# Ye-zixiao/Double-YOLO-Kaist

Measured on AMD Instinct MI355X. Metric: paired RGB+LWIR images/sec (train step), higher is better.
Workload: dtype bf16; 1 GPU; kaist_dyolov4_fshare_global_concat_se3.cfg train step (fwd+loss+bwd+Adam), 640x512 pairs, batch 16/GPU; global_batch=16, parallelism=dp1

## Files before the change

### double-yolo-kaist_amd/csrc/bn_act.hip

```cpp
#include <stdlib.h>
#include "dyk_common.h"

namespace {

__global__ __launch_bounds__(256) void bn_finalize_kernel(DykFinPair pr) {
    const DykBnFinalizeDesc d = pr.d[blockIdx.z];
    const int sub = threadIdx.x & 31;
    const int c = blockIdx.x * (blockDim.x >> 5) + (threadIdx.x >> 5);
    if (c >= d.C) return;
    const double n = (double)d.count;
    const int slots = d.slots > 0 ? d.slots : 1;
    double s1 = 0.0, s2 = 0.0;
    for (int r = sub; r < slots; r += 32) {
        double* st = d.stats + (size_t)r * 2 * d.C;
        s1 += st[c]; s2 += st[d.C + c];
        st[c] = 0.0; st[d.C + c] = 0.0;
    }
#pragma unroll
    for (int o = 16; o > 0; o >>= 1) { s1 += __shfl_xor(s1, o, 64); s2 += __shfl_xor(s2, o, 64); }
    if (sub != 0) return;
    const double mean = s1 / n;
    double var = s2 / n - mean * mean;
    if (var < 0.0) var = 0.0;
    const float rstd = (float)(1.0 / sqrt(var + (double)d.eps));
    const float g = d.gamma ? d.gamma[c] : 1.f, b = d.beta ? d.beta[c] : 0.f;
    const float sc = g * rstd;
    d.scale[c] = sc;
    d.shift[c] = b - (float)mean * sc;
    if (d.save_mean) d.save_mean[c] = (float)mean;
    if (d.save_rstd) d.save_rstd[c] = rstd;
    if (d.running_mean) {
        const double unb = n > 1.0 ? var * n / (n - 1.0) : var;
        d.running_mean[c] = (1.f - d.momentum) * d.running_mean[c] + d.momentum * (float)mean;
        d.running_var[c] = (1.f - d.momentum) * d.running_var[c] + d.momentum * (float)unb;
    }
}

__global__ void bn_fold_kernel(const float* gamma, const float* beta, const float* rm, const float* rv, float eps,
                               float* scale, float* shift, int C) {
    const int c = blockIdx.x * blockDim.x + threadIdx.x;
    if (c >= C) return;
    const float sc = (gamma ? gamma[c] : 1.f) / sqrtf(rv[c] + eps);
    scale[c] = sc;
    shift[c] = (beta ? beta[c] : 0.f) - rm[c] * sc;
}

template <typename T, int ACT>
__global__ __launch_bounds__(256) void bn_act_fwd_kernel(DykEwPair pr, int CVB) {
    const DykEwDesc d = pr.d[blockIdx.z];
    constexpr int EPV = ElemTraits<T>::EPV;
    const int PY = 256 / CVB;
    const int tx = threadIdx.x % CVB, ty = threadIdx.x / CVB;
    const int cv = blockIdx.x * CVB + tx;
    if (cv * EPV >= d.C) return;
    const int c = cv * EPV;
    float sc[EPV], sh[EPV];
#pragma unroll
    for (int j = 0; j < EPV; ++j) { sc[j] = d.p0 ? d.p0[c + j] : 1.f; sh[j] = d.p1 ? d.p1[c + j] : 0.f; }
    const T* __restrict__ a = (const T*)d.a;
    const T* __restrict__ r = (const T*)d.b;
    T* __restrict__ o = (T*)d.out;
    constexpr int U = 4;
    const long chunk = ((d.npix + gridDim.y - 1) / gridDim.y + PY - 1) / PY * PY;
    const long pend = min((long)d.npix, ((long)blockIdx.y + 1) * chunk);
    const long pstep = PY;
    for (long p0 = (long)blockIdx.y * chunk + ty; p0 < pend; p0 += pstep * U) {
        uint4 vx[U], vr[U];
#pragma unroll
        for (int u = 0; u < U; ++u) {
            const long p = p0 + u * pstep;
            if (p < pend) {
                vx[u] = ld_stream16(a + p * d.lda + c);
                if (r) vr[u] = *(const uint4*)(r + p * d.ldb + c);
            }
        }
#pragma unroll
        for (int u = 0; u < U; ++u) {
            const long p = p0 + u * pstep;
            if (p >= pend) break;
            float x[EPV], y[EPV];
            vec_unpack<T>(vx[u], x);
#pragma unroll
            for (int j = 0; j < EPV; ++j) y[j] = act_fwd_c<ACT>(x[j] * sc[j] + sh[j]);
            if (r) {
                float rr[EPV];
                vec_unpack<T>(vr[u], rr);
#pragma unroll
                for (int j = 0; j < EPV; ++j) y[j] += rr[j];
            }
            *(uint4*)(o + p * d.ldo + c) = vec_pack<T>(y);
        }
    }
}

template <typename T, int ACT>
__global__ __launch_bounds__(256) void bn_fused_fwd_kernel(DykFinPair fp, DykEwPair pr, int CVB) {
    const DykBnFinalizeDesc f = fp.d[blockIdx.z];
    const DykEwDesc d = pr.d[blockIdx.z];
    constexpr int EPV = ElemTraits<T>::EPV;
    __shared__ float s_aff[2][256];
    const int PY = 256 / CVB;
    const int tx = threadIdx.x % CVB, ty = threadIdx.x / CVB;
    const int cv = blockIdx.x * CVB + tx;
    {
        const int c_base = blockIdx.x * CVB * EPV;
        const int nch = min(CVB * EPV, d.C - c_base);
        const int slots = f.slots > 0 ? f.slots : 1;
        const size_t rs = (size_t)2 * f.C;
        for (int cl = threadIdx.x; cl < nch; cl += 256) {
            const int c = c_base + cl;
            constexpr int FB = 16;
            double a1[4] = {0.0, 0.0, 0.0, 0.0}, a2[4] = {0.0, 0.0, 0.0, 0.0};
            int r = 0;
            for (; r + FB <= slots; r += FB) {
                double v1[FB], v2[FB];
#pragma unroll
                for (int u = 0; u < FB; ++u) { v1[u] = f.stats[(size_t)(r + u) * rs + c]; v2[u] = f.stats[(size_t)(r + u) * rs + f.C + c]; }
#pragma unroll
                for (int u = 0; u < FB; ++u) { a1[u & 3] += v1[u]; a2[u & 3] += v2[u]; }
            }
            for (; r + 4 <= slots; r += 4) {
#pragma unroll
                for (int u = 0; u < 4; ++u) { a1[u] += f.stats[(size_t)(r + u) * rs + c]; a2[u] += f.stats[(size_t)(r + u) * rs + f.C + c]; }
            }
            for (; r < slots; ++r) { a1[0] += f.stats[(size_t)r * rs + c]; a2[0] += f.stats[(size_t)r * rs + f.C + c]; }
            const double n = (double)f.count;
            const double mean = ((a1[0] + a1[1]) + (a1[2] + a1[3])) / n;
            double var = ((a2[0] + a2[1]) + (a2[2] + a2[3])) / n - mean * mean;
            if (var < 0.0) var = 0.0;
            const float rstd = (float)(1.0 / sqrt(var + (double)f.eps));
            const float g = f.gamma ? f.gamma[c] : 1.f, b = f.beta ? f.beta[c] : 0.f;
            const float sc = g * rstd, sh = b - (float)mean * sc;
            s_aff[0][cl] = sc;
            s_aff[1][cl] = sh;
            if (blockIdx.y == 0) {
                f.scale[c] = sc;
                f.shift[c] = sh;
                if (f.save_mean) f.save_mean[c] = (float)mean;
                if (f.save_rstd) f.save_rstd[c] = rstd;
                if (f.running_mean) {
                    const double unb = n > 1.0 ? var * n / (n - 1.0) : var;
                    f.running_mean[c] = (1.f - f.momentum) * f.running_mean[c] + f.momentum * (float)mean;
                    f.running_var[c] = (1.f - f.momentum) * f.running_var[c] + f.momentum * (float)unb;
                }
            }
        }
        __syncthreads();
    }
    if (cv * EPV >= d.C) return;
    const int c = cv * EPV;
    float sc[EPV], sh[EPV];
#pragma unroll
    for (int j = 0; j < EPV; ++j) { sc[j] = s_aff[0][tx * EPV + j]; sh[j] = s_aff[1][tx * EPV + j]; }
    const T* __restrict__ a = (const T*)d.a;
    const T* __restrict__ r = (const T*)d.b;
    T* __restrict__ o = (T*)d.out;
    constexpr int U = 4;
    const long chunk = ((d.npix + gridDim.y - 1) / gridDim.y + PY - 1) / PY * PY;
    const long pend = min((long)d.npix, ((long)blockIdx.y + 1) * chunk);
    const long pstep = PY;
    for (long p0 = (long)blockIdx.y * chunk + ty; p0 < pend; p0 += pstep * U) {
        uint4 vx[U], vr[U];
#pragma unroll
        for (int u = 0; u < U; ++u) {
            const long p = p0 + u * pstep;
            if (p < pend) {
                vx[u] = ld_stream16(a + p * d.lda + c);
                if (r) vr[u] = *(const uint4*)(r + p * d.ldb + c);
            }
        }
#pragma unroll
        for (int u = 0; u < U; ++u) {
            const long p = p0 + u * pstep;
            if (p >= pend) break;
            float x[EPV], y[EPV];
            vec_unpack<T>(vx[u], x);
#pragma unroll
            for (int j = 0; j < EPV; ++j) y[j] = act_fwd_c<ACT>(x[j] * sc[j] + sh[j]);
            if (r) {
                float rr[EPV];
                vec_unpack<T>(vr[u], rr);
#pragma unroll
                for (int j = 0; j < EPV; ++j) y[j] += rr[j];
            }
            *(uint4*)(o + p * d.ldo + c) = vec_pack<T>(y);
        }
    }
}

template <typename T, int ACT>
__global__ __launch_bounds__(256) void bn_act_bwd_reduce_kernel(DykEwPair pr, int CVB) {
    const DykEwDesc d = pr.d[blockIdx.z];
    constexpr int EPV = ElemTraits<T>::EPV;
    __shared__ float red[256 * 2 * 8];
    const int PY = 256 / CVB;
    const int tx = threadIdx.x % CVB, ty = threadIdx.x / CVB;
    const int CV = d.C / EPV;
    const int cv = blockIdx.x * CVB + tx;
    const int c = cv * EPV;
    const bool active = cv < CV;
    float s1[EPV], s2[EPV];
#pragma unroll
    for (int j = 0; j < EPV; ++j) s1[j] = s2[j] = 0.f;
    if (active) {
        float sc[EPV], sh[EPV], mu[EPV], rs[EPV];
#pragma unroll
        for (int j = 0; j < EPV; ++j) {
            sc[j] = d.p0[c + j]; sh[j] = d.p1[c + j]; mu[j] = d.p2[c + j]; rs[j] = d.p3[c + j];
        }
        const T* __restrict__ dz = (const T*)d.a;
        const T* __restrict__ y = (const T*)d.b;
        constexpr int U = 4;
        const long chunk = ((d.npix + gridDim.y - 1) / gridDim.y + PY - 1) / PY * PY;
            const long pend = min((long)d.npix, ((long)blockIdx.y + 1) * chunk);
            const long pstep = PY;
            for (long p0 = (long)blockIdx.y * chunk + ty; p0 < pend; p0 += pstep * U) {
            uint4 vg[U], vy[U];
#pragma unroll
            for (int u = 0; u < U; ++u) {
                const long p = p0 + u * pstep;
                if (p < pend) { vg[u] = ld_stream16(dz + p * d.lda + c); vy[u] = ld_stream16(y + p * d.ldb + c); }
            }
#pragma unroll
            for (int u = 0; u < U; ++u) {
                if (p0 + u * pstep >= pend) break;
                float g[EPV], yy[EPV];
                vec_unpack<T>(vg[u], g);
                vec_unpack<T>(vy[u], yy);
#pragma unroll
                for (int j = 0; j < EPV; ++j) {
                    const float da = g[j] * act_bwd_c<ACT>(yy[j] * sc[j] + sh[j]);
                    s1[j] += da;
                    s2[j] += da * ((yy[j] - mu[j]) * rs[j]);
                }
            }
        }
    }
    float* mine = red + threadIdx.x * 2 * 8;
#pragma unroll
    for (int j = 0; j < EPV; ++j) { mine[j] = s1[j]; mine[8 + j] = s2[j]; }
    __syncthreads();
    if (ty == 0 && active) {
        for (int q = 1; q < PY; ++q) {
            const float* o = red + (q * CVB + tx) * 2 * 8;
#pragma unroll
            for (int j = 0; j < EPV; ++j) { s1[j] += o[j]; s2[j] += o[8 + j]; }
        }
        double* rd = d.red + (size_t)(blockIdx.y % (unsigned)(d.slots > 0 ? d.slots : 1)) * 2 * d.C;
#pragma unroll
        for (int j = 0; j < EPV; ++j) {
            atomicAdd(rd + c + j, (double)s1[j]);
            atomicAdd(rd + d.C + c + j, (double)s2[j]);
        }
    }
}

__global__ __launch_bounds__(256) void bn_bwd_params_kernel(double* red, float* dgamma, float* dbeta, int C, int slots) {
    const int sub = threadIdx.x & 31;
    const int c = blockIdx.x * (blockDim.x >> 5) + (threadIdx.x >> 5);
    if (c >= C) return;
    double s1 = 0.0, s2 = 0.0;
    for (int r = sub; r < slots; r += 32) { s1 += red[(size_t)r * 2 * C + c]; s2 += red[(size_t)r * 2 * C + C + c]; }
#pragma unroll
    for (int o = 16; o > 0; o >>= 1) { s1 += __shfl_xor(s1, o, 64); s2 += __shfl_xor(s2, o, 64); }
    if (sub != 0) return;
    red[c] = s1; red[C + c] = s2;
    if (dbeta) dbeta[c] += (float)s1;
    if (dgamma) dgamma[c] += (float)s2;
}

template <typename T, int ACT>
__global__ __launch_bounds__(256) void bn_act_bwd_apply_kernel(DykEwPair pr, int CVB) {
    const DykEwDesc d = pr.d[blockIdx.z];
    constexpr int EPV = ElemTraits<T>::EPV;
    __shared__ float s_tot[2][256];
    const int PY = 256 / CVB;
    const int tx = threadIdx.x % CVB, ty = threadIdx.x / CVB;
    const int cv = blockIdx.x * CVB + tx;
    {
        const int c_base = blockIdx.x * CVB * EPV;
        const int nch = min(CVB * EPV, d.C - c_base);
        const int slots = d.slots > 0 ? d.slots : 1;
        const size_t rs = d.H > 0 ? (size_t)d.H : (size_t)2 * d.C;
        const size_t so = d.W > 0 ? (size_t)d.W : (size_t)d.C;
        for (int cl = threadIdx.x; cl < nch; cl += 256) {
            const double* p = d.red + c_base + cl;
            double a8[2][8] = {{0.0, 0.0, 0.0, 0.0, 0.0, 0.0, 0.0, 0.0}, {0.0, 0.0, 0.0, 0.0, 0.0, 0.0, 0.0, 0.0}};
            int r = 0;
            for (; r + 16 <= slots; r += 16) {
                double v[2][16];
#pragma unroll
                for (int u = 0; u < 16; ++u) { v[0][u] = p[(size_t)(r + u) * rs]; v[1][u] = p[(size_t)(r + u) * rs + so]; }
#pragma unroll
                for (int u = 0; u < 16; ++u) { a8[0][u & 7] += v[0][u]; a8[1][u & 7] += v[1][u]; }
            }
            for (; r + 8 <= slots; r += 8) {
#pragma unroll
                for (int u = 0; u < 8; ++u) { a8[0][u] += p[(size_t)(r + u) * rs]; a8[1][u] += p[(size_t)(r + u) * rs + so]; }
            }
            for (; r < slots; ++r) { a8[0][0] += p[(size_t)r * rs]; a8[1][0] += p[(size_t)r * rs + so]; }
#pragma unroll
            for (int which = 0; which < 2; ++which) {
                const double acc = ((a8[which][0] + a8[which][1]) + (a8[which][2] + a8[which][3])) + ((a8[which][4] + a8[which][5]) + (a8[which][6] + a8[which][7]));
                s_tot[which][cl] = (float)acc;
                if (blockIdx.y == 0) {
                    float* g = which ? (float*)d.aux : (float*)d.aux2;
                    if (g) g[c_base + cl] += (float)acc;
                }
            }
        }
        __syncthreads();
    }
    if (cv * EPV >= d.C) return;
    const int c = cv * EPV;
    const float invn = 1.f / (float)d.npix;
    float sc[EPV], sh[EPV], mu[EPV], rs[EPV], m1[EPV], m2[EPV];
#pragma unroll
    for (int j = 0; j < EPV; ++j) {
        sc[j] = d.p0[c + j]; sh[j] = d.p1[c + j]; mu[j] = d.p2[c + j]; rs[j] = d.p3[c + j];
        m1[j] = s_tot[0][tx * EPV + j] * invn; m2[j] = s_tot[1][tx * EPV + j] * invn;
    }
    const T* __restrict__ dz = (const T*)d.a;
    const T* __restrict__ y = (const T*)d.b;
    T* __restrict__ o = (T*)d.out;
    const bool accum = d.flags & DYK_EW_ACCUM;
    constexpr int U = 4;
    const long chunk = ((d.npix + gridDim.y - 1) / gridDim.y + PY - 1) / PY * PY;
    const long pend = min((long)d.npix, ((long)blockIdx.y + 1) * chunk);
    const long pstep = PY;
    for (long p0 = (long)blockIdx.y * chunk + ty; p0 < pend; p0 += pstep * U) {
        uint4 vg[U], vy[U], vo[U];
#pragma unroll
        for (int u = 0; u < U; ++u) {
            const long p = p0 + u * pstep;
            if (p < pend) {
                vg[u] = ld_stream16(dz + p * d.lda + c);
                vy[u] = ld_stream16(y + p * d.ldb + c);
                if (accum) vo[u] = *(const uint4*)(o + p * d.ldo + c);
            }
        }
#pragma unroll
        for (int u = 0; u < U; ++u) {
            const long p = p0 + u * pstep;
            if (p >= pend) break;
            float g[EPV], yy[EPV], r[EPV];
            vec_unpack<T>(vg[u], g);
            vec_unpack<T>(vy[u], yy);
#pragma unroll
            for (int j = 0; j < EPV; ++j) {
                const float da = g[j] * act_bwd_c<ACT>(yy[j] * sc[j] + sh[j]);
                const float xh = (yy[j] - mu[j]) * rs[j];
                r[j] = sc[j] * (da - m1[j] - xh * m2[j]);
            }
            if (accum) {
                float old[EPV];
                vec_unpack<T>(vo[u], old);
#pragma unroll
                for (int j = 0; j < EPV; ++j) r[j] += old[j];
            }
            *(uint4*)(o + p * d.ldo + c) = vec_pack<T>(r);
        }
    }
}

inline int ew_grid2d(int CV, long npix, int* gx, int* gy) {
    int CVB = 1;
    while (CVB < CV && CVB < 32) CVB <<= 1;
    const int PY = 256 / CVB;
    *gx = (CV + CVB - 1) / CVB;
    constexpr int ppt = 8, capb = 2048;
    long g = (npix + (long)PY * ppt - 1) / ((long)PY * ppt);
    const long cap = capb / *gx > 0 ? capb / *gx : 1;
    if (g > cap) g = cap;
    if (g < 1) g = 1;
    *gy = (int)g;
    return CVB;
}

#define DYK_BN_LAUNCH_ACT(KERNEL, T, ...)                                                                         \
    switch (d->act) {                                                                                              \
    case DYK_ACT_LINEAR: hipLaunchKernelGGL((KERNEL<T, DYK_ACT_LINEAR>), __VA_ARGS__); break;                      \
    case DYK_ACT_LEAKY: hipLaunchKernelGGL((KERNEL<T, DYK_ACT_LEAKY>), __VA_ARGS__); break;                        \
    case DYK_ACT_MISH: hipLaunchKernelGGL((KERNEL<T, DYK_ACT_MISH>), __VA_ARGS__); break;                          \
    case DYK_ACT_RELU: hipLaunchKernelGGL((KERNEL<T, DYK_ACT_RELU>), __VA_ARGS__); break;                          \
    case DYK_ACT_RELU6: hipLaunchKernelGGL((KERNEL<T, DYK_ACT_RELU6>), __VA_ARGS__); break;                        \
    case DYK_ACT_HSIGMOID: hipLaunchKernelGGL((KERNEL<T, DYK_ACT_HSIGMOID>), __VA_ARGS__); break;                  \
    case DYK_ACT_HSWISH: hipLaunchKernelGGL((KERNEL<T, DYK_ACT_HSWISH>), __VA_ARGS__); break;                      \
    default: return DYK_ERR_ARG;                                                                                   \
    }
#define DYK_BN_LAUNCH(KERNEL, ...)                                        \
    if (d->dtype == DYK_BF16) { DYK_BN_LAUNCH_ACT(KERNEL, bf16_t, __VA_ARGS__) } \
    else { DYK_BN_LAUNCH_ACT(KERNEL, float, __VA_ARGS__) }

inline int ew_check(const DykEwDesc* d, bool need_b) {
    if (!d || !d->a || !d->out || d->npix <= 0 || d->C <= 0) return DYK_ERR_ARG;
    if (need_b && !d->b) return DYK_ERR_ARG;
    const int epv = d->dtype == DYK_BF16 ? 8 : 4;
    if (d->dtype != DYK_BF16 && d->dtype != DYK_F32) return DYK_ERR_ARG;
    if (d->C % epv || d->lda % epv || d->ldo % epv || (d->b && d->ldb % epv)) return DYK_ERR_ARG;
    return DYK_OK;
}

}

extern "C" int dyk_bn_finalize(const DykBnFinalizeDesc* d, void* stream) {
    if (!d || !d->stats || !d->scale || !d->shift || d->C <= 0 || d->count <= 0) return DYK_ERR_ARG;
    DykFinPair fp;
    const int nz = dyk_fill_fin_pair(fp, d);
    if (!nz) return DYK_ERR_ARG;
    hipLaunchKernelGGL(bn_finalize_kernel, dim3((d->C + 7) / 8, 1, nz), dim3(256), 0, (hipStream_t)stream, fp);
    DYK_LAUNCH_CHECK();
    return DYK_OK;
}

extern "C" int dyk_bn_fold(const float* gamma, const float* beta, const float* running_mean,
                           const float* running_var, float eps, float* scale, float* shift, int32_t C,
                           void* stream) {
    if (!running_mean || !running_var || !scale || !shift || C <= 0) return DYK_ERR_ARG;
    hipLaunchKernelGGL(bn_fold_kernel, dim3((C + 127) / 128), dim3(128), 0, (hipStream_t)stream, gamma, beta,
                       running_mean, running_var, eps, scale, shift, C);
    DYK_LAUNCH_CHECK();
    return DYK_OK;
}

extern "C" int dyk_bn_act_fwd(const DykEwDesc* d, void* stream) {
    const int rc = ew_check(d, false);
    if (rc) return rc;
    const int epv = d->dtype == DYK_BF16 ? 8 : 4;
    int gx, gy;
    const int CVB = ew_grid2d(d->C / epv, d->npix, &gx, &gy);
    DykEwPair pr;
    const int nz = dyk_fill_ew_pair(pr, d);
    if (!nz) return DYK_ERR_ARG;
    DYK_BN_LAUNCH(bn_act_fwd_kernel, dim3(gx, gy, nz), dim3(256), 0, (hipStream_t)stream, pr, CVB)
    DYK_LAUNCH_CHECK();
    return DYK_OK;
}

extern "C" int dyk_bn_finalize_act_fwd(const DykBnFinalizeDesc* f, const DykEwDesc* d, void* stream) {
    if (!f || !f->stats || !f->scale || !f->shift || f->C <= 0 || f->count <= 0) return DYK_ERR_ARG;
    const int rc = ew_check(d, false);
    if (rc) return rc;
    if (d->C != f->C) return DYK_ERR_ARG;
    const int epv = d->dtype == DYK_BF16 ? 8 : 4;
    int gx, gy;
    const int CVB = ew_grid2d(d->C / epv, d->npix, &gx, &gy);
    DykEwPair pr;
    DykFinPair fp;
    const int nz = dyk_fill_ew_pair(pr, d);
    if (!nz || dyk_fill_fin_pair(fp, f) != nz) return DYK_ERR_ARG;
    DYK_BN_LAUNCH(bn_fused_fwd_kernel, dim3(gx, gy, nz), dim3(256), 0, (hipStream_t)stream, fp, pr, CVB)
    DYK_LAUNCH_CHECK();
    return DYK_OK;
}

extern "C" int dyk_bn_act_bwd_reduce(const DykEwDesc* d, void* stream) {
    if (!d || !d->a || !d->b || !d->red || !d->p0 || !d->p1 || !d->p2 || !d->p3) return DYK_ERR_ARG;
    if (d->npix <= 0 || d->C <= 0 || (d->dtype != DYK_BF16 && d->dtype != DYK_F32)) return DYK_ERR_ARG;
    const int epv = d->dtype == DYK_BF16 ? 8 : 4;
    if (d->C % epv || d->lda % epv || d->ldb % epv) return DYK_ERR_ARG;
    const int CV = d->C / epv;
    int CVB = 1;
    while (CVB < CV && CVB < 32) CVB <<= 1;
    const int PY = 256 / CVB;
    const int gx = (CV + CVB - 1) / CVB;
    long gy = ((long)d->npix + PY * 8 - 1) / (PY * 8);
    const long cap = 2048 / gx > 0 ? 2048 / gx : 1;
    if (gy > cap) gy = cap;
    if (gy < 1) gy = 1;
    DykEwPair pr;
    const int nz = dyk_fill_ew_pair(pr, d);
    if (!nz) return DYK_ERR_ARG;
    DYK_BN_LAUNCH(bn_act_bwd_reduce_kernel, dim3(gx, (int)gy, nz), dim3(256), 0, (hipStream_t)stream, pr, CVB)
    DYK_LAUNCH_CHECK();
    return DYK_OK;
}

extern "C" int dyk_bn_bwd_params(double* red, float* dgamma, float* dbeta, int32_t C, int32_t slots, void* stream) {
    if (!red || C <= 0) return DYK_ERR_ARG;
    hipLaunchKernelGGL(bn_bwd_params_kernel, dim3((C + 7) / 8), dim3(256), 0, (hipStream_t)stream, red, dgamma, dbeta, C,
                       slots > 0 ? slots : 1);
    DYK_LAUNCH_CHECK();
    return DYK_OK;
}

extern "C" int dyk_bn_act_bwd_apply(const DykEwDesc* d, void* stream) {
    const int rc = ew_check(d, true);
    if (rc) return rc;
    if (d->flags & DYK_EW_SKIP) return DYK_OK;
    if (!d->red || !d->p0 || !d->p1 || !d->p2 || !d->p3) return DYK_ERR_ARG;
    const int epv = d->dtype == DYK_BF16 ? 8 : 4;
    int gx, gy;
    const int CVB = ew_grid2d(d->C / epv, d->npix, &gx, &gy);
    DykEwPair pr;
    const int nz = dyk_fill_ew_pair(pr, d);
    if (!nz) return DYK_ERR_ARG;
    DYK_BN_LAUNCH(bn_act_bwd_apply_kernel, dim3(gx, gy, nz), dim3(256), 0, (hipStream_t)stream, pr, CVB)
    DYK_LAUNCH_CHECK();
    return DYK_OK;
}
```

Measured before the change: 583.1 pairs/s.

## Split BN stat replica folding across lanes and prefetch activations before finalize

In the fused BN finalize+activation forward kernel and the BN backward apply kernel, the per-channel reduction over stat replica slots is now spread across several lanes per channel (chosen at launch as 8, 4 or 1), with partial sums combined by cross-lane shuffles. When multiple lanes are used, the first activation tile loads, and in backward the per-channel parameters, are issued before the slot reduction so their latency overlaps it. The main loop is restructured into a request/compute pipeline that prefetches the next tile. The aim is to shorten the serial prologue in which only a few threads walked all slots, at the cost of more template variants, higher register pressure from the in-flight loads, and a changed floating-point summation order.

New measurement: 584.2 pairs/s (median of 3 runs). No clear change (+0.2%).

```diff
diff --git a/double-yolo-kaist_amd/csrc/bn_act.hip b/double-yolo-kaist_amd/csrc/bn_act.hip
--- a/double-yolo-kaist_amd/csrc/bn_act.hip
+++ b/double-yolo-kaist_amd/csrc/bn_act.hip
@@ -93,7 +93,72 @@
     }
 }
 
-template <typename T, int ACT>
+template <int NCH, int L, int NB>
+__device__ __forceinline__ void fold_batch(const double* __restrict__ p, size_t rs, size_t so, int r, uint32_t lo, double (&a)[2][NCH / L]) {
+    constexpr int K = NCH / L, PB = NB / NCH;
+    double v[2][K][PB];
+#pragma unroll
+    for (int i = 0; i < PB; ++i)
+#pragma unroll
+        for (int k = 0; k < K; ++k) {
+            const double* pr = p + (size_t)(r + i * NCH + k * L) * rs;
+            v[0][k][i] = pr[lo]; v[1][k][i] = (pr + so)[lo];
+        }
+#pragma unroll
+    for (int i = 0; i < PB; ++i)
+#pragma unroll
+        for (int k = 0; k < K; ++k) { a[0][k] += v[0][k][i]; a[1][k] += v[1][k][i]; }
+}
+
+template <int L>
+__device__ __forceinline__ void fold_lane(size_t rs, int& cl, int& q, uint32_t& lo) {
+    constexpr int CW = 64 / L;
+    const int lane = threadIdx.x & 63;
+    q = lane / CW;
+    cl = (threadIdx.x >> 6) * CW + lane % CW;
+    lo = (uint32_t)cl + (uint32_t)q * (uint32_t)rs;
+    if constexpr (L > 1) asm volatile("" : "+v"(lo));
+}
+
+template <int NCH, int L, int FB>
+__device__ __forceinline__ void fold_replicas(const double* __restrict__ p, size_t rs, size_t so, int slots, uint32_t lo, int q, bool live,
+                                              double& t0, double& t1) {
+    static_assert(NCH % L == 0 && FB % NCH == 0 && FB / NCH <= 8, "chains per lane, batches of whole rounds of the chains");
+    constexpr int K = NCH / L;
+    double a[2][K];
+#pragma unroll
+    for (int k = 0; k < K; ++k) a[0][k] = a[1][k] = 0.0;
+    if (live) {
+        const int whole = slots & ~(NCH - 1);
+        int r = 0;
+        if constexpr (L > 1) {
+            if (FB <= whole) {
+                fold_batch<NCH, L, FB>(p, rs, so, 0, lo, a);
+                for (r = FB; r + FB <= whole; r += FB) fold_batch<NCH, L, FB>(p, rs, so, r, lo, a);
+            }
+        } else {
+            for (; r + FB <= whole; r += FB) fold_batch<NCH, L, FB>(p, rs, so, r, lo, a);
+        }
+        if constexpr (FB / 2 >= NCH) if (r + FB / 2 <= whole) { fold_batch<NCH, L, FB / 2>(p, rs, so, r, lo, a); r += FB / 2; }
+        if constexpr (FB / 4 >= NCH) if (r + FB / 4 <= whole) { fold_batch<NCH, L, FB / 4>(p, rs, so, r, lo, a); r += FB / 4; }
+        if constexpr (FB / 8 >= NCH) if (r + FB / 8 <= whole) { fold_batch<NCH, L, FB / 8>(p, rs, so, r, lo, a); r += FB / 8; }
+        if (q == 0)
+            for (; r < slots; ++r) { a[0][0] += (p + (size_t)r * rs)[lo]; a[1][0] += (p + (size_t)r * rs + so)[lo]; }
+    }
+#pragma unroll
+    for (int m = 1; m < NCH; m <<= 1) {
+        if (m < L) {
+#pragma unroll
+            for (int k = 0; k < K; ++k) { a[0][k] += __shfl_xor(a[0][k], m * (64 / L), 64); a[1][k] += __shfl_xor(a[1][k], m * (64 / L), 64); }
+        } else {
+#pragma unroll
+            for (int k = 0; k < K; k += 2 * (m / L)) { a[0][k] += a[0][k + m / L]; a[1][k] += a[1][k + m / L]; }
+        }
+    }
+    t0 = a[0][0]; t1 = a[1][0];
+}
+
+template <typename T, int ACT, int L>
 __global__ __launch_bounds__(256) void bn_fused_fwd_kernel(DykFinPair fp, DykEwPair pr, int CVB) {
     const DykBnFinalizeDesc f = fp.d[blockIdx.z];
     const DykEwDesc d = pr.d[blockIdx.z];
@@ -102,56 +167,11 @@
     const int PY = 256 / CVB;
     const int tx = threadIdx.x % CVB, ty = threadIdx.x / CVB;
     const int cv = blockIdx.x * CVB + tx;
-    {
-        const int c_base = blockIdx.x * CVB * EPV;
-        const int nch = min(CVB * EPV, d.C - c_base);
-        const int slots = f.slots > 0 ? f.slots : 1;
-        const size_t rs = (size_t)2 * f.C;
-        for (int cl = threadIdx.x; cl < nch; cl += 256) {
-            const int c = c_base + cl;
-            constexpr int FB = 16;
-            double a1[4] = {0.0, 0.0, 0.0, 0.0}, a2[4] = {0.0, 0.0, 0.0, 0.0};
-            int r = 0;
-            for (; r + FB <= slots; r += FB) {
-                double v1[FB], v2[FB];
-#pragma unroll
-                for (int u = 0; u < FB; ++u) { v1[u] = f.stats[(size_t)(r + u) * rs + c]; v2[u] = f.stats[(size_t)(r + u) * rs + f.C + c]; }
-#pragma unroll
-                for (int u = 0; u < FB; ++u) { a1[u & 3] += v1[u]; a2[u & 3] += v2[u]; }
-            }
-            for (; r + 4 <= slots; r += 4) {
-#pragma unroll
-                for (int u = 0; u < 4; ++u) { a1[u] += f.stats[(size_t)(r + u) * rs + c]; a2[u] += f.stats[(size_t)(r + u) * rs + f.C + c]; }
-            }
-            for (; r < slots; ++r) { a1[0] += f.stats[(size_t)r * rs + c]; a2[0] += f.stats[(size_t)r * rs + f.C + c]; }
-            const double n = (double)f.count;
-            const double mean = ((a1[0] + a1[1]) + (a1[2] + a1[3])) / n;
-            double var = ((a2[0] + a2[1]) + (a2[2] + a2[3])) / n - mean * mean;
-            if (var < 0.0) var = 0.0;
-            const float rstd = (float)(1.0 / sqrt(var + (double)f.eps));
-            const float g = f.gamma ? f.gamma[c] : 1.f, b = f.beta ? f.beta[c] : 0.f;
-            const float sc = g * rstd, sh = b - (float)mean * sc;
-            s_aff[0][cl] = sc;
-            s_aff[1][cl] = sh;
-            if (blockIdx.y == 0) {
-                f.scale[c] = sc;
-                f.shift[c] = sh;
-                if (f.save_mean) f.save_mean[c] = (float)mean;
-                if (f.save_rstd) f.save_rstd[c] = rstd;
-                if (f.running_mean) {
-                    const double unb = n > 1.0 ? var * n / (n - 1.0) : var;
-                    f.running_mean[c] = (1.f - f.momentum) * f.running_mean[c] + f.momentum * (float)mean;
-                    f.running_var[c] = (1.f - f.momentum) * f.running_var[c] + f.momentum * (float)unb;
-                }
-            }
-        }
-        __syncthreads();
-    }
-    if (cv * EPV >= d.C) return;
     const int c = cv * EPV;
-    float sc[EPV], sh[EPV];
-#pragma unroll
-    for (int j = 0; j < EPV; ++j) { sc[j] = s_aff[0][tx * EPV + j]; sh[j] = s_aff[1][tx * EPV + j]; }
+    const bool active = c < d.C;
+    int cl, q;
+    uint32_t lo;
+    fold_lane<L>((size_t)2 * f.C, cl, q, lo);
     const T* __restrict__ a = (const T*)d.a;
     const T* __restrict__ r = (const T*)d.b;
     T* __restrict__ o = (T*)d.out;
@@ -159,8 +179,9 @@
     const long chunk = ((d.npix + gridDim.y - 1) / gridDim.y + PY - 1) / PY * PY;
     const long pend = min((long)d.npix, ((long)blockIdx.y + 1) * chunk);
     const long pstep = PY;
-    for (long p0 = (long)blockIdx.y * chunk + ty; p0 < pend; p0 += pstep * U) {
-        uint4 vx[U], vr[U];
+    long p0 = (long)blockIdx.y * chunk + ty;
+    uint4 vx[U], vr[U];
+    auto request = [&]() {
 #pragma unroll
         for (int u = 0; u < U; ++u) {
             const long p = p0 + u * pstep;
@@ -169,6 +190,53 @@
                 if (r) vr[u] = *(const uint4*)(r + p * d.ldb + c);
             }
         }
+    };
+    constexpr bool early = L > 1;
+    if (early && active) request();
+    {
+        const int c_base = blockIdx.x * CVB * EPV;
+        const int nch = min(CVB * EPV, d.C - c_base);
+        const int slots = f.slots > 0 ? f.slots : 1;
+        const bool live = cl < nch;
+        const int cf = c_base + cl;
+        float g = 1.f, b = 0.f;
+        float rm = 0.f, rv = 0.f;
+        if (live && q == 0) {
+            if (f.gamma) g = f.gamma[cf];
+            if (f.beta) b = f.beta[cf];
+            if (blockIdx.y == 0 && f.running_mean) { rm = f.running_mean[cf]; rv = f.running_var[cf]; }
+        }
+        double t1, t2;
+        fold_replicas<4, L, (L == 1 ? 16 : 32)>(f.stats + c_base, (size_t)2 * f.C, (size_t)f.C, slots, lo, q, live, t1, t2);
+        if (live && q == 0) {
+            const double n = (double)f.count;
+            const double mean = t1 / n;
+            double var = t2 / n - mean * mean;
+            if (var < 0.0) var = 0.0;
+            const float rstd = (float)(1.0 / sqrt(var + (double)f.eps));
+            const float sc = g * rstd, sh = b - (float)mean * sc;
+            s_aff[0][cl] = sc;
+            s_aff[1][cl] = sh;
+            if (blockIdx.y == 0) {
+                f.scale[cf] = sc;
+                f.shift[cf] = sh;
+                if (f.save_mean) f.save_mean[cf] = (float)mean;
+                if (f.save_rstd) f.save_rstd[cf] = rstd;
+                if (f.running_mean) {
+                    const double unb = n > 1.0 ? var * n / (n - 1.0) : var;
+                    f.running_mean[cf] = (1.f - f.momentum) * rm + f.momentum * (float)mean;
+                    f.running_var[cf] = (1.f - f.momentum) * rv + f.momentum * (float)unb;
+                }
+            }
+        }
+        __syncthreads();
+    }
+    if (!active) return;
+    float sc[EPV], sh[EPV];
+#pragma unroll
+    for (int j = 0; j < EPV; ++j) { sc[j] = s_aff[0][tx * EPV + j]; sh[j] = s_aff[1][tx * EPV + j]; }
+    if (!early) request();
+    while (p0 < pend) {
 #pragma unroll
         for (int u = 0; u < U; ++u) {
             const long p = p0 + u * pstep;
@@ -185,6 +253,8 @@
             }
             *(uint4*)(o + p * d.ldo + c) = vec_pack<T>(y);
         }
+        p0 += pstep * U;
+        request();
     }
 }
 
@@ -269,7 +339,7 @@
     if (dgamma) dgamma[c] += (float)s2;
 }
 
-template <typename T, int ACT>
+template <typename T, int ACT, int L>
 __global__ __launch_bounds__(256) void bn_act_bwd_apply_kernel(DykEwPair pr, int CVB) {
     const DykEwDesc d = pr.d[blockIdx.z];
     constexpr int EPV = ElemTraits<T>::EPV;
@@ -277,49 +347,13 @@
     const int PY = 256 / CVB;
     const int tx = threadIdx.x % CVB, ty = threadIdx.x / CVB;
     const int cv = blockIdx.x * CVB + tx;
-    {
-        const int c_base = blockIdx.x * CVB * EPV;
-        const int nch = min(CVB * EPV, d.C - c_base);
-        const int slots = d.slots > 0 ? d.slots : 1;
-        const size_t rs = d.H > 0 ? (size_t)d.H : (size_t)2 * d.C;
-        const size_t so = d.W > 0 ? (size_t)d.W : (size_t)d.C;
-        for (int cl = threadIdx.x; cl < nch; cl += 256) {
-            const double* p = d.red + c_base + cl;
-            double a8[2][8] = {{0.0, 0.0, 0.0, 0.0, 0.0, 0.0, 0.0, 0.0}, {0.0, 0.0, 0.0, 0.0, 0.0, 0.0, 0.0, 0.0}};
-            int r = 0;
-            for (; r + 16 <= slots; r += 16) {
-                double v[2][16];
-#pragma unroll
-                for (int u = 0; u < 16; ++u) { v[0][u] = p[(size_t)(r + u) * rs]; v[1][u] = p[(size_t)(r + u) * rs + so]; }
-#pragma unroll
-                for (int u = 0; u < 16; ++u) { a8[0][u & 7] += v[0][u]; a8[1][u & 7] += v[1][u]; }
-            }
-            for (; r + 8 <= slots; r += 8) {
-#pragma unroll
-                for (int u = 0; u < 8; ++u) { a8[0][u] += p[(size_t)(r + u) * rs]; a8[1][u] += p[(size_t)(r + u) * rs + so]; }
-            }
-            for (; r < slots; ++r) { a8[0][0] += p[(size_t)r * rs]; a8[1][0] += p[(size_t)r * rs + so]; }
-#pragma unroll
-            for (int which = 0; which < 2; ++which) {
-                const double acc = ((a8[which][0] + a8[which][1]) + (a8[which][2] + a8[which][3])) + ((a8[which][4] + a8[which][5]) + (a8[which][6] + a8[which][7]));
-                s_tot[which][cl] = (float)acc;
-                if (blockIdx.y == 0) {
-                    float* g = which ? (float*)d.aux : (float*)d.aux2;
-                    if (g) g[c_base + cl] += (float)acc;
-                }
-            }
-        }
-        __syncthreads();
-    }
-    if (cv * EPV >= d.C) return;
     const int c = cv * EPV;
-    const float invn = 1.f / (float)d.npix;
-    float sc[EPV], sh[EPV], mu[EPV], rs[EPV], m1[EPV], m2[EPV];
-#pragma unroll
-    for (int j = 0; j < EPV; ++j) {
-        sc[j] = d.p0[c + j]; sh[j] = d.p1[c + j]; mu[j] = d.p2[c + j]; rs[j] = d.p3[c + j];
-        m1[j] = s_tot[0][tx * EPV + j] * invn; m2[j] = s_tot[1][tx * EPV + j] * invn;
-    }
+    const bool active = c < d.C;
+    const size_t rstride = d.H > 0 ? (size_t)d.H : (size_t)2 * d.C;
+    const size_t so = d.W > 0 ? (size_t)d.W : (size_t)d.C;
+    int cl, q;
+    uint32_t lo;
+    fold_lane<L>(rstride, cl, q, lo);
     const T* __restrict__ dz = (const T*)d.a;
     const T* __restrict__ y = (const T*)d.b;
     T* __restrict__ o = (T*)d.out;
@@ -328,8 +362,9 @@
     const long chunk = ((d.npix + gridDim.y - 1) / gridDim.y + PY - 1) / PY * PY;
     const long pend = min((long)d.npix, ((long)blockIdx.y + 1) * chunk);
     const long pstep = PY;
-    for (long p0 = (long)blockIdx.y * chunk + ty; p0 < pend; p0 += pstep * U) {
-        uint4 vg[U], vy[U], vo[U];
+    long p0 = (long)blockIdx.y * chunk + ty;
+    uint4 vg[U], vy[U], vo[U];
+    auto request = [&]() {
 #pragma unroll
         for (int u = 0; u < U; ++u) {
             const long p = p0 + u * pstep;
@@ -339,6 +374,50 @@
                 if (accum) vo[u] = *(const uint4*)(o + p * d.ldo + c);
             }
         }
+    };
+    constexpr bool early = L > 1;
+    float sc[EPV], sh[EPV], mu[EPV], rs[EPV];
+    if (active) {
+        if constexpr (early) {
+#pragma unroll
+            for (int j = 0; j < EPV; ++j) { sc[j] = d.p0[c + j]; sh[j] = d.p1[c + j]; mu[j] = d.p2[c + j]; rs[j] = d.p3[c + j]; }
+            request();
+        }
+    }
+    {
+        const int c_base = blockIdx.x * CVB * EPV;
+        const int nch = min(CVB * EPV, d.C - c_base);
+        const int slots = d.slots > 0 ? d.slots : 1;
+        const bool live = cl < nch;
+        float* const gsum[2] = {(float*)d.aux2, (float*)d.aux};
+        float gold[2] = {0.f, 0.f};
+        if (live && q == 0 && blockIdx.y == 0) {
+#pragma unroll
+            for (int which = 0; which < 2; ++which)
+                if (gsum[which]) gold[which] = gsum[which][c_base + cl];
+        }
+        double acc[2];
+        fold_replicas<8, L, 16>(d.red + c_base, rstride, so, slots, lo, q, live, acc[0], acc[1]);
+        if (live && q == 0) {
+#pragma unroll
+            for (int which = 0; which < 2; ++which) {
+                s_tot[which][cl] = (float)acc[which];
+                if (blockIdx.y == 0 && gsum[which]) gsum[which][c_base + cl] = gold[which] + (float)acc[which];
+            }
+        }
+        __syncthreads();
+    }
+    if (!active) return;
+    const float invn = 1.f / (float)d.npix;
+    if constexpr (!early) {
+#pragma unroll
+        for (int j = 0; j < EPV; ++j) { sc[j] = d.p0[c + j]; sh[j] = d.p1[c + j]; mu[j] = d.p2[c + j]; rs[j] = d.p3[c + j]; }
+    }
+    float m1[EPV], m2[EPV];
+#pragma unroll
+    for (int j = 0; j < EPV; ++j) { m1[j] = s_tot[0][tx * EPV + j] * invn; m2[j] = s_tot[1][tx * EPV + j] * invn; }
+    if (!early) request();
+    while (p0 < pend) {
 #pragma unroll
         for (int u = 0; u < U; ++u) {
             const long p = p0 + u * pstep;
@@ -360,6 +439,8 @@
             }
             *(uint4*)(o + p * d.ldo + c) = vec_pack<T>(r);
         }
+        p0 += pstep * U;
+        request();
     }
 }
 
@@ -391,6 +472,27 @@
 #define DYK_BN_LAUNCH(KERNEL, ...)                                        \
     if (d->dtype == DYK_BF16) { DYK_BN_LAUNCH_ACT(KERNEL, bf16_t, __VA_ARGS__) } \
     else { DYK_BN_LAUNCH_ACT(KERNEL, float, __VA_ARGS__) }
+#define DYK_BN_LAUNCH_ACT_L(KERNEL, T, LANES, ...)                                                                 \
+    switch (d->act) {                                                                                              \
+    case DYK_ACT_LINEAR: hipLaunchKernelGGL((KERNEL<T, DYK_ACT_LINEAR, LANES>), __VA_ARGS__); break;               \
+    case DYK_ACT_LEAKY: hipLaunchKernelGGL((KERNEL<T, DYK_ACT_LEAKY, LANES>), __VA_ARGS__); break;                 \
+    case DYK_ACT_MISH: hipLaunchKernelGGL((KERNEL<T, DYK_ACT_MISH, LANES>), __VA_ARGS__); break;                   \
+    case DYK_ACT_RELU: hipLaunchKernelGGL((KERNEL<T, DYK_ACT_RELU, LANES>), __VA_ARGS__); break;                   \
+    case DYK_ACT_RELU6: hipLaunchKernelGGL((KERNEL<T, DYK_ACT_RELU6, LANES>), __VA_ARGS__); break;                 \
+    case DYK_ACT_HSIGMOID: hipLaunchKernelGGL((KERNEL<T, DYK_ACT_HSIGMOID, LANES>), __VA_ARGS__); break;           \
+    case DYK_ACT_HSWISH: hipLaunchKernelGGL((KERNEL<T, DYK_ACT_HSWISH, LANES>), __VA_ARGS__); break;               \
+    default: return DYK_ERR_ARG;                                                                                   \
+    }
+#define DYK_BN_LAUNCH_L(KERNEL, LANES, ...)                                                 \
+    if (d->dtype == DYK_BF16) { DYK_BN_LAUNCH_ACT_L(KERNEL, bf16_t, LANES, __VA_ARGS__) }   \
+    else { DYK_BN_LAUNCH_ACT_L(KERNEL, float, LANES, __VA_ARGS__) }
+
+inline int fold_lanes(int CVB, int epv, int C, int chains) {
+    const int nch = CVB * epv < C ? CVB * epv : C;
+    int L = chains;
+    while (L > 2 && nch * L > 256) L >>= 1;
+    return nch * L <= 256 && L > 2 ? L : 1;
+}
 
 inline int ew_check(const DykEwDesc* d, bool need_b) {
     if (!d || !d->a || !d->out || d->npix <= 0 || d->C <= 0) return DYK_ERR_ARG;
@@ -449,7 +551,10 @@
     DykFinPair fp;
     const int nz = dyk_fill_ew_pair(pr, d);
     if (!nz || dyk_fill_fin_pair(fp, f) != nz) return DYK_ERR_ARG;
-    DYK_BN_LAUNCH(bn_fused_fwd_kernel, dim3(gx, gy, nz), dim3(256), 0, (hipStream_t)stream, fp, pr, CVB)
+    switch (fold_lanes(CVB, epv, d->C, 4)) {
+    case 4: DYK_BN_LAUNCH_L(bn_fused_fwd_kernel, 4, dim3(gx, gy, nz), dim3(256), 0, (hipStream_t)stream, fp, pr, CVB) break;
+    default: DYK_BN_LAUNCH_L(bn_fused_fwd_kernel, 1, dim3(gx, gy, nz), dim3(256), 0, (hipStream_t)stream, fp, pr, CVB) break;
+    }
     DYK_LAUNCH_CHECK();
     return DYK_OK;
 }
@@ -495,7 +600,11 @@
     DykEwPair pr;
     const int nz = dyk_fill_ew_pair(pr, d);
     if (!nz) return DYK_ERR_ARG;
-    DYK_BN_LAUNCH(bn_act_bwd_apply_kernel, dim3(gx, gy, nz), dim3(256), 0, (hipStream_t)stream, pr, CVB)
+    switch (fold_lanes(CVB, epv, d->C, 8)) {
+    case 8: DYK_BN_LAUNCH_L(bn_act_bwd_apply_kernel, 8, dim3(gx, gy, nz), dim3(256), 0, (hipStream_t)stream, pr, CVB) break;
+    case 4: DYK_BN_LAUNCH_L(bn_act_bwd_apply_kernel, 4, dim3(gx, gy, nz), dim3(256), 0, (hipStream_t)stream, pr, CVB) break;
+    default: DYK_BN_LAUNCH_L(bn_act_bwd_apply_kernel, 1, dim3(gx, gy, nz), dim3(256), 0, (hipStream_t)stream, pr, CVB) break;
+    }
     DYK_LAUNCH_CHECK();
     return DYK_OK;
 }
```
